# privacy-scaling-explorations/snark-verifier

Hardware: AMD Instinct MI355X
Metric: BN254 G1 MSM points/sec at 2^20 (higher is better)
Workload: dtype i32x9 (254-bit Montgomery Fq as 9 x 29-bit limbs on the integer VALU)

## Files before the change

snark-verifier_amd/csrc/ctx.hpp:

```cpp
#pragma once
#include <hip/hip_runtime.h>
#include <stddef.h>
#include <stdint.h>
#include <stdio.h>
#include "../../include/snarkv_amd.h"
#include "curve_consts.h"

#if defined(SNARKV_CURVE_PALLAS)
#define SNARKV_API(name) snarkv_pallas_##name
#else
#define SNARKV_API(name) snarkv_##name
#endif

namespace snarkv {

void set_last_error(const char* fmt, ...);

#define SNARKV_HIP(expr)                                                                   \
  do {                                                                                     \
    hipError_t _e = (expr);                                                                \
    if (_e != hipSuccess) {                                                                \
      ::snarkv::set_last_error("%s:%d: %s -> %s", __FILE__, __LINE__, #expr, hipGetErrorString(_e)); \
      return SNARKV_ERR_DEVICE;                                                            \
    }                                                                                      \
  } while (0)

#define SNARKV_TRY(expr)      \
  do {                        \
    int _rc = (expr);         \
    if (_rc < 0) return _rc;  \
  } while (0)

enum Slot {
  SLOT_IN_SCALARS = 0,
  SLOT_IN_POINTS,
  SLOT_IN_OFFSETS,
  SLOT_OUT,
  SLOT_POINTS_MONT,
  SLOT_COUNTS,
  SLOT_OFFSETS,
  SLOT_CURSOR,
  SLOT_BLOCKSUMS,
  SLOT_ENTRIES,
  SLOT_SEG_IDS,
  SLOT_SEG_PARTIALS,
  SLOT_BUCKETS,
  SLOT_CHUNK_PARTIALS,
  SLOT_WINDOW_SUMS,
  SLOT_TERM_PARTIALS,
  SLOT_FLAGS,
  SLOT_MISC,
  SLOT_SORT_TMP,
  SLOT_SHIFTED,
  SLOT_GLV,
  SLOT_BIG_LIST,
  SLOT_MISC2,
  SLOT_TERM_CHAIN,
  SLOT_TERM_MAGS,
  SLOT_SPLIT_PARTIALS,
  SLOT_IPA_XI,
  SLOT_IPA_H,
  SLOT_IPA_OUT,
  SLOT_MGPU_GRID,
  SLOT_MGPU_RECV,
  SLOT_COUNT
};

}

struct snarkv_ctx {
  int device;
  hipStream_t stream;
  bool own_stream;
  void* buf[snarkv::SLOT_COUNT];
  size_t cap[snarkv::SLOT_COUNT];
  void* hbuf[SNARKV_HOST_BUFFERS];
  size_t hbuf_cap[SNARKV_HOST_BUFFERS];
  uint32_t flags;
  bool mont;
  bool stage_timing;
  float stage_ms[SNARKV_PIP_STAGES];
  hipEvent_t ev[SNARKV_PIP_STAGES + 1];
  bool ev_ready;
  snarkv_ctx* sub[4];
  hipEvent_t sub_ev[5];
  bool sub_ready;
  hipEvent_t sorted_ev;
  bool sorted_ev_ready;
  int last_split_workers;
  bool throughput_mode;
  int throughput_peers;
  bool is_lane;
  snarkv_ctx* jobs[SNARKV_MANY_MAX_JOBS];
  int njobs;
  int last_many_jobs;
  size_t many_sig;
  hipStream_t copy_stream;
  bool copy_ready;
  hipEvent_t many_ev[2];
  hipEvent_t order_ev;
  bool order_ev_ready;
  hipStream_t hi_stream[2];
  bool hi_ready;
};

struct snarkv_dk {
  int device;
  void* d_prep;
// ... 66 lines not shown
```

snark-verifier_amd/csrc/msm_pippenger.hip:

```cpp
#include <stdlib.h>
#include <string.h>
#include <algorithm>
#include <mutex>
#include <atomic>
#include "ctx.hpp"
#include "g1_29.h"
#include "fr29.h"
#ifndef SNARKV_GLV
#define SNARKV_GLV 1
#endif
#if SNARKV_GLV
#include "glv.h"
#endif

namespace snarkv {

#ifndef SNARKV_KRUN
#define SNARKV_KRUN 64
#endif
#ifndef SNARKV_KCHUNK
#define SNARKV_KCHUNK 8
#endif
#ifndef SNARKV_TILE_THREADS
#define SNARKV_TILE_THREADS 256
#endif
#ifndef SNARKV_SCATTER_ATTR
#define SNARKV_SCATTER_ATTR __attribute__((amdgpu_waves_per_eu(5)))
#endif
#ifndef SNARKV_L2_THREADS
#define SNARKV_L2_THREADS 512
#endif
#ifndef SNARKV_LEVEL2_ATTR
#define SNARKV_LEVEL2_ATTR
#endif
#ifndef SNARKV_PREP_THREADS
#define SNARKV_PREP_THREADS SNARKV_TILE_THREADS
#endif
#ifndef SNARKV_XCD_TILES
#define SNARKV_XCD_TILES 1
#endif
#ifndef SNARKV_TILE_BASE
#define SNARKV_TILE_BASE 2048
#endif
#ifndef SNARKV_ACC_WAVES
#define SNARKV_ACC_WAVES 3
#endif
#ifndef SNARKV_BPRIO
#define SNARKV_BPRIO 3
#endif
#define SNARKV_RAISE_PRIO() __builtin_amdgcn_s_setprio(SNARKV_BPRIO)

constexpr int kHalves = SNARKV_GLV ? 2 : 1;
constexpr int kDigitWords = SNARKV_GLV ? 4 : 8;
constexpr int kDigitBits = 32 * kDigitWords;
constexpr int kRun = SNARKV_KRUN;
#ifndef SNARKV_KRUN_THROUGHPUT
#define SNARKV_KRUN_THROUGHPUT 96
#endif
constexpr int kRunThroughput = SNARKV_KRUN_THROUGHPUT;
constexpr int kChunk = SNARKV_KCHUNK;
constexpr uint32_t kSortCap = 7168;
constexpr uint32_t kSortTarget = 3072;
constexpr uint32_t kMaxKeys = 16384;
constexpr uint32_t kBigSpan = 24;
constexpr uint32_t kBigGrid = 8192;
constexpr uint32_t kMaxBig = 8192;
constexpr uint32_t kNoBucket = 0xFFFFFFFFu;

struct PipParams {
  uint32_t n;
  int c;
  int W;
  uint32_t B;
  uint32_t nb;
  int low_bits;
  uint32_t SB;
  uint32_t nkeys;
  uint32_t nblk;
  uint32_t tile;
  uint32_t mstride;
  uint32_t w0;
  uint32_t krun;
  uint32_t wper;
  uint32_t chunk_log2;
  uint32_t mont;
};

__device__ __forceinline__ uint32_t half_bits(const uint32_t (&k)[kDigitWords], int lo, int c) {
  if (lo >= kDigitBits) return 0;
  int word = lo >> 5, sh = lo & 31;
  uint32_t w0 = 0u, w1 = 0u;
#pragma unroll
  for (int i = 0; i < kDigitWords; ++i) {
    w0 = word == i ? k[i] : w0;
    if (i > 0) w1 = word == i - 1 ? k[i] : w1;
  }
  uint64_t v = ((uint64_t)w1 << 32) | w0;
  return (uint32_t)(v >> sh) & ((1u << c) - 1u);
}

template <class F>
__device__ __forceinline__ void for_each_digit(const uint32_t (&k)[kDigitWords], uint32_t sgn, const PipParams& p, F emit) {
  uint32_t carry = 0;
  for (int w = 0; w < p.W; ++w) {
    uint32_t raw = half_bits(k, w * p.c, p.c) + carry;
    uint32_t neg = raw > p.B ? 1u : 0u;
    uint32_t d = neg ? ((1u << p.c) - raw) : raw;
    carry = neg;
    if (d != 0) emit((uint32_t)w * p.SB + ((d - 1) >> p.low_bits), (uint32_t)w * p.B + d - 1, neg ^ sgn);
  }
}
template <class F>
__device__ __forceinline__ void digit_of_window(const uint32_t (&k)[kDigitWords], uint32_t sgn, const PipParams& p, int w,
                                                F emit) {
  uint32_t carry = 0;
  for (int j = w - 1; j >= 0; --j) {
    uint32_t b = half_bits(k, j * p.c, p.c);
    if (b != p.B) {
      carry = b > p.B ? 1u : 0u;
      break;
// ... 256 lines not shown
  SNARKV_RAISE_PRIO();
  extern __shared__ uint32_t lds[];
  const uint32_t nbins = 1u << p.low_bits;
  uint32_t* hist = lds;
  uint32_t* scan = lds + nbins;
  uint2* stage = reinterpret_cast<uint2*>(lds + nbins + SNARKV_L2_THREADS + (nbins & 1u));
  const uint32_t T = blockDim.x;
  uint32_t key = blockIdx.x;
  uint32_t begin = M[(size_t)key * p.mstride];
  uint32_t end = (key + 1 < p.nkeys) ? M[(size_t)(key + 1) * p.mstride] : misc[0];
  uint32_t cnt_items = end - begin;
  bool fast = cnt_items <= kSortCap;
  for (uint32_t k = threadIdx.x; k < nbins; k += T) hist[k] = 0;
  __syncthreads();
  const uint32_t low_mask = nbins - 1;
  constexpr int kPer = kSortCap / SNARKV_L2_THREADS;
  static_assert(kSortCap % SNARKV_L2_THREADS == 0, "kSortCap items spread evenly over the lanes");
  uint2 mine[kPer];
  if (fast) {
#pragma unroll
    for (int j = 0; j < kPer; ++j) {
      uint32_t e = threadIdx.x + j * T;
      if (e < cnt_items) {
        mine[j] = tmp[begin + e];
        atomicAdd(&hist[mine[j].x & low_mask], 1u);
      }
    }
  } else {
    for (uint32_t e = begin + threadIdx.x; e < end; e += T) atomicAdd(&hist[tmp[e].x & low_mask], 1u);
  }
  __syncthreads();
  uint32_t per = (nbins + T - 1) / T;
  uint32_t s0 = threadIdx.x * per;
  uint32_t sum = 0;
  for (uint32_t k = s0; k < s0 + per && k < nbins; ++k) sum += hist[k];
  scan[threadIdx.x] = sum;
  __syncthreads();
  for (uint32_t off = 1; off < T; off <<= 1) {
    uint32_t t = (threadIdx.x >= off) ? scan[threadIdx.x - off] : 0;
    __syncthreads();
    scan[threadIdx.x] += t;
    __syncthreads();
  }
  uint32_t run = scan[threadIdx.x] - sum;
  uint32_t w = key / p.SB, sb = key % p.SB;
  uint32_t bucket0 = w * p.B + (sb << p.low_bits);
  for (uint32_t k = s0; k < s0 + per && k < nbins; ++k) {
    uint32_t cnt = hist[k];
    counts[bucket0 + k] = cnt;
    offsets[bucket0 + k] = begin + run;
    hist[k] = run;
    run += cnt;
  }
  if (key == p.nkeys - 1 && threadIdx.x == 0) misc[4] = 0u;
  __syncthreads();
  if (fast) {
#pragma unroll
    for (int j = 0; j < kPer; ++j) {
      uint32_t e = threadIdx.x + j * T;
      if (e < cnt_items) stage[atomicAdd(&hist[mine[j].x & low_mask], 1u)] = mine[j];
    }
    __syncthreads();
    for (uint32_t e = threadIdx.x; e < cnt_items; e += T) entries[begin + e] = stage[e];
  } else {
    for (uint32_t e = begin + threadIdx.x; e < end; e += T) {
      uint2 it = tmp[e];
      entries[begin + atomicAdd(&hist[it.x & low_mask], 1u)] = it;
    }
  }
}

constexpr uint32_t kEntryIdx = 0x7FFFFFFFu;

__device__ __forceinline__ G1Affine29 entry_point(const G1Packed& k, uint32_t y) {
  G1Affine29 p = g1a29_unpack(k);
  if (y >> 31) p.y = fq29_neg(p.y);
  return p;
}

template <int RUN>
__global__ void __launch_bounds__(64, SNARKV_ACC_WAVES)
    k_accumulate(const uint2* __restrict__ entries, const uint32_t* __restrict__ total_ptr,
                 const G1Packed* __restrict__ pts, G1Xyzz29* __restrict__ buckets, uint32_t* __restrict__ seg_ids,
                 G1Xyzz29* __restrict__ seg_parts) {
  const uint32_t t = blockIdx.x * blockDim.x + threadIdx.x;
  const uint32_t stop = *total_ptr;
  const uint64_t begin64 = (uint64_t)t * RUN;
  if (begin64 >= stop) return;
  const uint32_t begin = (uint32_t)begin64;
  const uint32_t end = (stop - begin > (uint32_t)RUN) ? begin + RUN : stop;
  const size_t slot = t;
  uint32_t cur = entries[begin].x;
  bool first = true, fresh = true;
  G1Xyzz29 acc = xyzz29_identity();
  auto flush = [&]() {
    if (first) {
      seg_ids[2 * slot] = cur;
      seg_parts[2 * slot] = acc;
      first = false;
    } else {
      buckets[cur] = acc;
    }
  };
  auto step = [&](const uint2& ent, const G1Packed& pk) {
    if (ent.x != cur) {
      flush();
      cur = ent.x;
      fresh = true;
    }
    G1Affine29 p = entry_point(pk, ent.y);
    if (fresh) {
      acc.x = p.x;
      acc.y = p.y;
      acc.zz = fq29_one();
      acc.zzz = fq29_one();
      fresh = false;
    } else {
      xyzz29_madd_fast(acc, p);
    }
  };
  uint2 ent0 = entries[begin], ent1 = ent0;
  G1Packed p0 = pts[ent0.y & kEntryIdx], p1 = p0;
#pragma unroll 1
  for (uint32_t e = begin; e < end; e += 2) {
    if (e + 1 < end) {
      ent1 = entries[e + 1];
      p1 = pts[ent1.y & kEntryIdx];
    }
    step(ent0, p0);
    if (e + 1 < end) {
      if (e + 2 < end) {
        ent0 = entries[e + 2];
        p0 = pts[ent0.y & kEntryIdx];
      }
      step(ent1, p1);
    }
  }
  if (first) {
    seg_ids[2 * slot] = cur;
    seg_parts[2 * slot] = acc;
    seg_ids[2 * slot + 1] = kNoBucket;
  } else {
    seg_ids[2 * slot + 1] = cur;
    seg_parts[2 * slot + 1] = acc;
  }
}

__device__ __noinline__ void bucket_from_entries_careful(const uint2* __restrict__ entries, const G1Packed* __restrict__ pts,
                                                         uint32_t o, uint32_t cnt, uint32_t first, uint32_t stride,
                                                         bool sanitize, G1Xyzz29* out) {
  G1Xyzz29 acc = xyzz29_identity();
  for (uint32_t e = o + first; e < o + cnt; e += stride) {
    uint2 ent = entries[e];
    G1Affine29 p = entry_point(pts[ent.y & kEntryIdx], ent.y);
    xyzz29_madd_careful(acc, p);
  }
  *out = sanitize ? xyzz29_sanitize(acc) : acc;
}

__device__ __forceinline__ void run_span(const PipParams& p, uint32_t o, uint32_t cnt, size_t& s0, size_t& s1) {
  s0 = o / p.krun;
  s1 = (o + cnt - 1) / p.krun;
}

__global__ void __launch_bounds__(64)
    k_combine(const uint32_t* __restrict__ counts, const uint32_t* __restrict__ offsets, PipParams p,
              const uint2* __restrict__ entries, const G1Packed* __restrict__ pts,
              const uint32_t* __restrict__ seg_ids, const G1Xyzz29* __restrict__ seg_parts,
              G1Xyzz29* __restrict__ buckets, uint32_t* __restrict__ big_count, uint32_t* __restrict__ big_list) {
  SNARKV_RAISE_PRIO();
  uint32_t b = blockIdx.x * blockDim.x + threadIdx.x;
  if (b >= p.nb) return;
  uint32_t cnt = counts[b];
  if (cnt == 0) {
    buckets[b] = xyzz29_identity();
    return;
  }
  uint32_t o = offsets[b];
  size_t s0, s1;
  run_span(p, o, cnt, s0, s1);
  if (s1 - s0 >= kBigSpan) {
    uint32_t slot = atomicAdd(big_count, 1u);
    if (slot < kMaxBig) {
      big_list[slot] = b;
      return;
    }
  }
  G1Xyzz29 acc = xyzz29_identity();
  bool touched = false, bad = false;
  for (size_t s = s0; s <= s1; ++s) {
    for (int h = 0; h < 2; ++h) {
      if (seg_ids[2 * s + h] == b) {
        G1Xyzz29 part = seg_parts[2 * s + h];
        bad = bad || xyzz29_is_identity(part);
        xyzz29_add_skipid_fast(acc, part, bad);
        touched = true;
      }
    }
  }
  if (!touched) acc = buckets[b];
  bad = bad || xyzz29_is_degenerate(acc);
  if (bad) bucket_from_entries_careful(entries, pts, o, cnt, 0, 1, true, &buckets[b]);
  else if (touched) buckets[b] = acc;
}

__global__ void __launch_bounds__(256)
    k_combine_big(const uint32_t* __restrict__ counts, const uint32_t* __restrict__ offsets,
                  const uint2* __restrict__ entries, const G1Packed* __restrict__ pts,
                  const uint32_t* __restrict__ seg_ids, const G1Xyzz29* __restrict__ seg_parts,
                  G1Xyzz29* __restrict__ buckets, const uint32_t* __restrict__ big_count,
                  const uint32_t* __restrict__ big_list, PipParams p) {
  SNARKV_RAISE_PRIO();
  __shared__ G1Xyzz29 sh[256];
  __shared__ int any_bad;
  uint32_t nbig = *big_count < kMaxBig ? *big_count : kMaxBig;
  for (uint32_t bi = blockIdx.x; bi < nbig; bi += gridDim.x) {
    uint32_t b = big_list[bi];
    uint32_t o = offsets[b], cnt = counts[b];
    size_t s0, s1;
    run_span(p, o, cnt, s0, s1);
    if (threadIdx.x == 0) any_bad = 0;
    __syncthreads();
    G1Xyzz29 acc = xyzz29_identity();
    bool bad = false;
    for (size_t s = s0 + threadIdx.x; s <= s1; s += 256)
      for (int h = 0; h < 2; ++h)
        if (seg_ids[2 * s + h] == b) {
          G1Xyzz29 part = seg_parts[2 * s + h];
          bad = bad || xyzz29_is_degenerate(part);
          xyzz29_add_careful(acc, part);
        }
    if (bad) atomicOr(&any_bad, 1);
    __syncthreads();
    if (any_bad) bucket_from_entries_careful(entries, pts, o, cnt, threadIdx.x, 256, false, &sh[threadIdx.x]);
    else sh[threadIdx.x] = acc;
    __syncthreads();
    for (uint32_t st = 128; st >= 1; st >>= 1) {
      if (threadIdx.x < st) {
        G1Xyzz29 a = sh[threadIdx.x];
        xyzz29_add_careful(a, sh[threadIdx.x + st]);
        sh[threadIdx.x] = a;
      }
      __syncthreads();
    }
    if (threadIdx.x == 0) buckets[b] = xyzz29_sanitize(sh[0]);
    __syncthreads();
  }
}

__device__ __forceinline__ G1Xyzz29 xyzz29_sel(bool c, const G1Xyzz29& a, const G1Xyzz29& b) {
  G1Xyzz29 r;
#pragma unroll
  for (int i = 0; i < 9; ++i) {
    r.x.v[i] = c ? a.x.v[i] : b.x.v[i];
    r.y.v[i] = c ? a.y.v[i] : b.y.v[i];
    r.zz.v[i] = c ? a.zz.v[i] : b.zz.v[i];
    r.zzz.v[i] = c ? a.zzz.v[i] : b.zzz.v[i];
  }
  return r;
}

template <bool CAREFUL>
__device__ __forceinline__ bool chunk_sums(const G1Xyzz29* __restrict__ bw, uint32_t base, uint32_t top,
                                           G1Xyzz29& run, G1Xyzz29& acc) {
  run = xyzz29_identity();
  acc = xyzz29_identity();
  bool bad = false;
#pragma unroll 1
  for (uint32_t op = 0; op < 2 * (top - base); ++op) {
    bool second = op & 1u;
    G1Xyzz29 x = second ? acc : run;
    G1Xyzz29 y = second ? run : bw[top - 1 - (op >> 1)];
    if (CAREFUL) xyzz29_add_careful(x, y);
    else xyzz29_add_skipid_fast(x, y, bad);
    if (second) acc = x;
    else run = x;
  }
  if (CAREFUL) return false;
  return bad || (!xyzz29_is_identity(run) && xyzz29_is_degenerate(run)) ||
         (!xyzz29_is_identity(acc) && xyzz29_is_degenerate(acc));
}

__device__ __forceinline__ void wave_weighted_fold(G1Xyzz29* sh, const G1Xyzz29& run, const G1Xyzz29& acc,
                                                   const G1Xyzz29& extra, int log2_l, int log2_scale,
                                                   G1Xyzz29& out, G1Xyzz29* total_dst) {
  const uint32_t lane = threadIdx.x;
  G1Xyzz29 x = run;
#pragma unroll 1
  for (int step = 0; step < 14; ++step) {
    sh[lane] = x;
    __syncthreads();
    G1Xyzz29 y;
    int ndbl = 0;
    if (step == 6) {
      if (lane == 0 && total_dst) *total_dst = sh[0];
      x = xyzz29_sel(lane >= 1, x, xyzz29_identity());
      y = acc;
      ndbl = log2_l;
    } else if (step == 7) {
// ... 102 lines not shown
    }
    __syncthreads();
  }
  if (lane == 0) {
    if (partial_out) {
      *reinterpret_cast<G1Xyzz29*>(out) = sh[0];
    } else {
      G1Affine29 r = xyzz29_to_affine(sh[0]);
      uint32_t w[16];
      g1a29_to_words(r, w, mont != 0);
      for (int i = 0; i < 16; ++i) out[i] = w[i];
    }
  }
}

int launch_fold_partials_many(snarkv_ctx* ctx, const void* d_partials, size_t count, size_t jobs, void* d_out64s) {
  hipLaunchKernelGGL(k_final, dim3((uint32_t)jobs), dim3(64), 0, ctx->stream, (const G1Xyzz29*)d_partials, (uint32_t)count,
                     (uint32_t*)d_out64s, 0, ctx->mont ? 1u : 0u);
  SNARKV_HIP(hipGetLastError());
  return SNARKV_OK;
}

int launch_fold_partials(snarkv_ctx* ctx, const void* d_partials, size_t count, void* d_out64, bool partial_out) {
  hipLaunchKernelGGL(k_final, dim3(1), dim3(64), 0, ctx->stream, (const G1Xyzz29*)d_partials, (uint32_t)count,
                     (uint32_t*)d_out64, partial_out ? 1 : 0, ctx->mont ? 1u : 0u);
  SNARKV_HIP(hipGetLastError());
  return SNARKV_OK;
}

static int default_window_bits(size_t n) {
  int best = 2;
  double best_cost = 0;
  for (int c = 2; c <= 22; ++c) {
    const int W = (kDigitBits + c - 1) / c;
    const int top = kDigitBits - 1 - (W - 1) * c;
    double cost = (double)kHalves * (double)n * W * 10.0 + (double)W * (double)(1u << (c - 1)) * 30.0;
    if (top < c - 3) cost *= 1.6;
    if (c == 2 || cost < best_cost) best = c, best_cost = cost;
  }
  return best;
}

static int balance_window_bits(int c) {
  int W = (kDigitBits + c - 1) / c;
  return (kDigitBits + W - 1) / W;
}

static uint32_t latency_run_length(uint64_t entries) {
  auto waves = [&](uint64_t run) { return (entries + 64 * run - 1) / (64 * run); };
  if (waves(16) <= 4608) return waves(16) >= 2048 ? 16u : 32u;
  if (waves(32) <= 4608) return 32u;
  return (uint32_t)kRun;
}

int launch_msm_pippenger(snarkv_ctx* ctx, const void* d_scalars, const void* d_points, size_t n, int window_bits,
                         void* d_out, bool partial_out, void* d_buckets_out) {
  return launch_msm_pippenger_phases(ctx, ctx->stream, PIP_PHASE_ALL, d_scalars, d_points, n, window_bits, d_out,
                                     partial_out, d_buckets_out, nullptr);
}

int launch_msm_pippenger_phases(snarkv_ctx* ctx, hipStream_t st, int phases, const void* d_scalars, const void* d_points,
                                size_t n, int window_bits, void* d_out, bool partial_out, void* d_buckets_out,
                                void* d_grid) {
  PipParams p;
  p.w0 = 0;
  p.wper = 0;
  p.chunk_log2 = (uint32_t)kLog2Chunk;
  p.mont = ctx->mont ? 1u : 0u;
  p.n = (uint32_t)n;
  p.c = window_bits > 0 ? window_bits : balance_window_bits(default_window_bits(n));
  if (p.c < 2) p.c = 2;
  if (p.c > 22) p.c = 22;
  p.W = (kDigitBits + p.c - 1) / p.c;
  p.B = 1u << (p.c - 1);
  p.nb = (uint32_t)p.W * p.B;
  int high = p.c - 1 > 10 ? p.c - 1 - 10 : 0;
  while (high < p.c - 1 && ((kHalves * n) >> (high + 1)) >= kSortTarget && ((uint64_t)p.W << (high + 1)) <= kMaxKeys) ++high;
  p.low_bits = (p.c - 1) - high;
  p.SB = p.B >> p.low_bits;
  p.nkeys = (uint32_t)p.W * p.SB;
  p.tile = SNARKV_TILE_BASE;
  static_assert(kStageItems * kHalves <= 32, "a staged lane keeps one sign bit per entry in a 32-bit word");
  const size_t lds_staged = ((size_t)3 * p.SB + 16 + (p.SB & 1u)) * 4 + (size_t)kStageScalars * kHalves * 8;
  p.nblk = (uint32_t)((n + p.tile - 1) / p.tile);
  p.mstride = p.nblk | 1u;
  uint64_t max_entries = (uint64_t)kHalves * (uint64_t)n * (uint64_t)p.W;
  if (n == 0 || max_entries >= 0xFFFFFFFFull || n >= 0x40000000ull) {
    set_last_error("pippenger: n=%zu out of range", n);
    return SNARKV_ERR_LENGTH;
  }
  if ((size_t)p.nkeys * 4 > 65536 || lds_staged > 96 * 1024) {
    set_last_error("pippenger: key table too large (nkeys=%u)", p.nkeys);
    return SNARKV_ERR_LENGTH;
  }
  p.krun = ctx->throughput_mode ? (uint32_t)kRunThroughput : latency_run_length(max_entries);
  const uint32_t max_runs = (uint32_t)((max_entries + p.krun - 1) / p.krun) + 1;
  uint32_t mcount = p.nkeys * p.mstride;
  uint32_t scan_blocks = (mcount + 1023) / 1024;
  uint32_t chunks_per_window = (p.B + kChunk - 1) / kChunk;
  uint32_t blocks_per_window = (chunks_per_window + 63) / 64;

  void *d_pts, *d_glv, *d_counts, *d_offsets, *d_M, *d_blocksum, *d_entries, *d_tmp, *d_seg_ids, *d_seg_parts,
      *d_buckets, *d_wave, *d_shift, *d_misc, *d_big;
  SNARKV_TRY(ctx_reserve(ctx, SLOT_POINTS_MONT, kHalves * n * sizeof(G1Packed), &d_pts));
  SNARKV_TRY(ctx_reserve(ctx, SLOT_GLV, n * 32, &d_glv));
  SNARKV_TRY(ctx_reserve(ctx, SLOT_COUNTS, (size_t)p.nb * 4, &d_counts));
  SNARKV_TRY(ctx_reserve(ctx, SLOT_OFFSETS, (size_t)p.nb * 4, &d_offsets));
  SNARKV_TRY(ctx_reserve(ctx, SLOT_CURSOR, (size_t)mcount * 4, &d_M));
  SNARKV_TRY(ctx_reserve(ctx, SLOT_BLOCKSUMS, (size_t)scan_blocks * 4 + 64, &d_blocksum));
  SNARKV_TRY(ctx_reserve(ctx, SLOT_ENTRIES, max_entries * 8, &d_entries));
  SNARKV_TRY(ctx_reserve(ctx, SLOT_SORT_TMP, max_entries * 8, &d_tmp));
  SNARKV_TRY(ctx_reserve(ctx, SLOT_SEG_IDS, (size_t)max_runs * 8, &d_seg_ids));
  SNARKV_TRY(ctx_reserve(ctx, SLOT_SEG_PARTIALS, (size_t)max_runs * 2 * sizeof(G1Xyzz29), &d_seg_parts));
  if (d_grid) d_buckets = d_grid;
  else SNARKV_TRY(ctx_reserve(ctx, SLOT_BUCKETS, (size_t)p.nb * sizeof(G1Xyzz29), &d_buckets));
  SNARKV_TRY(ctx_reserve(ctx, SLOT_CHUNK_PARTIALS, 2 * (size_t)blocks_per_window * p.W * sizeof(G1Xyzz29), &d_wave));
  SNARKV_TRY(ctx_reserve(ctx, SLOT_SHIFTED, (size_t)p.W * sizeof(G1Xyzz29), &d_shift));
  SNARKV_TRY(ctx_reserve(ctx, SLOT_MISC, 64, &d_misc));
  SNARKV_TRY(ctx_reserve(ctx, SLOT_BIG_LIST, (size_t)kMaxBig * 4, &d_big));
  uint32_t* d_total = (uint32_t*)d_misc;
  uint32_t* d_big_count = d_total + 4;

  const bool tm = ctx->stage_timing && phases == PIP_PHASE_ALL;
  const bool tm_acc = ctx->stage_timing && phases == PIP_PHASE_ACC;
  int evi = 0;
#define STAGE_MARK()                                         \
  do {                                                       \
    if (tm) SNARKV_HIP(hipEventRecord(ctx->ev[evi++], st));  \
  } while (0)
  if ((tm || tm_acc) && !ctx->ev_ready) {
    for (int i = 0; i <= SNARKV_PIP_STAGES; ++i) SNARKV_HIP(hipEventCreate(&ctx->ev[i]));
    ctx->ev_ready = true;
  }
  STAGE_MARK();
  if (phases & PIP_PHASE_SORT) {
    hipLaunchKernelGGL(k_prepare, dim3(p.nblk), dim3(SNARKV_PREP_THREADS), (size_t)p.nkeys * 4, st, (const uint32_t*)d_scalars,
                       (const uint32_t*)d_points, (G1Packed*)d_pts, (uint4*)d_glv, p, (uint32_t*)d_M);
    STAGE_MARK();
    hipLaunchKernelGGL(k_scan_local, dim3(scan_blocks), dim3(256), 0, st, (uint32_t*)d_M, (uint32_t*)d_blocksum, mcount);
    hipLaunchKernelGGL(k_scan_blocksums, dim3(1), dim3(1024), 0, st, (uint32_t*)d_blocksum, scan_blocks, d_total);
    hipLaunchKernelGGL(k_scan_add, dim3(scan_blocks), dim3(256), 0, st, (uint32_t*)d_M, (const uint32_t*)d_blocksum,
                       mcount);
    STAGE_MARK();
    static std::atomic<uint64_t> attr_set{0};
    const uint64_t bit = 1ull << (ctx->device & 63);
    if (!(attr_set.load(std::memory_order_relaxed) & bit)) {
      SNARKV_HIP(hipFuncSetAttribute(reinterpret_cast<const void*>(k_sort_scatter_staged),
                                     hipFuncAttributeMaxDynamicSharedMemorySize, 96 * 1024));
      attr_set.fetch_or(bit, std::memory_order_relaxed);
    }
    hipLaunchKernelGGL(k_sort_scatter_staged, dim3(p.nblk), dim3(SNARKV_TILE_THREADS), lds_staged, st, (const uint4*)d_glv,
                       p, (const uint32_t*)d_M, (uint2*)d_tmp);
    const uint32_t nbins_l2 = 1u << p.low_bits;
    const size_t lds2 = ((size_t)nbins_l2 + SNARKV_L2_THREADS + 1) * 4 + (size_t)kSortCap * 8;
    hipLaunchKernelGGL(k_sort_level2, dim3(p.nkeys), dim3(SNARKV_L2_THREADS), lds2, st, (const uint2*)d_tmp, (const uint32_t*)d_M,
                       d_total, p, (uint2*)d_entries, (uint32_t*)d_counts, (uint32_t*)d_offsets);
  }
  STAGE_MARK();
  if (tm_acc) SNARKV_HIP(hipEventRecord(ctx->ev[3], st));
  if (phases & PIP_PHASE_ACC) {
    auto acc_kernel = p.krun == 16u ? k_accumulate<16> : p.krun == 32u ? k_accumulate<32>
                      : p.krun == (uint32_t)kRun ? k_accumulate<kRun> : k_accumulate<kRunThroughput>;
    hipLaunchKernelGGL(acc_kernel, dim3((max_runs + 63) / 64), dim3(64), 0, st, (const uint2*)d_entries,
                       (const uint32_t*)d_total, (const G1Packed*)d_pts, (G1Xyzz29*)d_buckets, (uint32_t*)d_seg_ids,
                       (G1Xyzz29*)d_seg_parts);
  }
  STAGE_MARK();
  if (tm_acc) SNARKV_HIP(hipEventRecord(ctx->ev[4], st));
  if (phases & PIP_PHASE_ACC) {
    hipLaunchKernelGGL(k_combine, dim3((p.nb + 63) / 64), dim3(64), 0, st, (const uint32_t*)d_counts,
                       (const uint32_t*)d_offsets, p, (const uint2*)d_entries, (const G1Packed*)d_pts,
                       (const uint32_t*)d_seg_ids, (const G1Xyzz29*)d_seg_parts, (G1Xyzz29*)d_buckets, d_big_count,
                       (uint32_t*)d_big);
    const uint32_t big_grid = std::min<uint32_t>(max_runs / kBigSpan + 1, kBigGrid);
    hipLaunchKernelGGL(k_combine_big, dim3(big_grid), dim3(256), 0, st, (const uint32_t*)d_counts,
                       (const uint32_t*)d_offsets, (const uint2*)d_entries, (const G1Packed*)d_pts,
                       (const uint32_t*)d_seg_ids, (const G1Xyzz29*)d_seg_parts, (G1Xyzz29*)d_buckets,
                       (const uint32_t*)d_big_count, (const uint32_t*)d_big, p);
    if (tm_acc) SNARKV_HIP(hipEventRecord(ctx->ev[5], st));
  }
  STAGE_MARK();
  if (d_buckets_out) {
    if (phases & PIP_PHASE_ACC)
      SNARKV_HIP(hipMemcpyAsync(d_buckets_out, d_buckets, (size_t)p.nb * sizeof(G1Xyzz29), hipMemcpyDeviceToDevice, st));
    SNARKV_HIP(hipGetLastError());
    return SNARKV_OK;
  }
  if (phases & PIP_PHASE_TAIL)
    hipLaunchKernelGGL(k_bucket_reduce, dim3(blocks_per_window * p.W), dim3(64), 0, st, (const G1Xyzz29*)d_buckets,
                       (G1Xyzz29*)d_wave, p, chunks_per_window, blocks_per_window);
  STAGE_MARK();
  if (phases & PIP_PHASE_TAIL)
    hipLaunchKernelGGL(k_shift_windows, dim3(p.W), dim3(64), 0, st, (const G1Xyzz29*)d_wave, (G1Xyzz29*)d_shift, p,
                       blocks_per_window);
  STAGE_MARK();
  if (phases & PIP_PHASE_TAIL)
    hipLaunchKernelGGL(k_final, dim3(1), dim3(64), 0, st, (const G1Xyzz29*)d_shift, (uint32_t)p.W, (uint32_t*)d_out,
                       partial_out ? 1 : 0, p.mont);
  STAGE_MARK();
#undef STAGE_MARK
  SNARKV_HIP(hipGetLastError());
  return SNARKV_OK;
}

int pip_geometry(size_t n_total, int window_bits, uint32_t* c, uint32_t* windows, uint32_t* buckets_per_window) {
  int cc = window_bits > 0 ? window_bits : balance_window_bits(default_window_bits(n_total));
  if (cc < 2) cc = 2;
  if (cc > 22) cc = 22;
  *c = (uint32_t)cc;
  *windows = (uint32_t)((kDigitBits + cc - 1) / cc);
  *buckets_per_window = 1u << (cc - 1);
  return SNARKV_OK;
}

__global__ void __launch_bounds__(256) k_buckets_add(G1Xyzz29* __restrict__ dst, const G1Xyzz29* __restrict__ src, uint32_t count) {
  SNARKV_RAISE_PRIO();
  uint32_t i = blockIdx.x * blockDim.x + threadIdx.x;
  if (i >= count) return;
  G1Xyzz29 a = dst[i];
  xyzz29_add_careful(a, src[i]);
  dst[i] = xyzz29_sanitize(a);
}

int launch_buckets_add(snarkv_ctx* ctx, void* d_dst, const void* d_src, size_t count) {
  hipLaunchKernelGGL(k_buckets_add, dim3((uint32_t)((count + 255) / 256)), dim3(256), 0, ctx->stream, (G1Xyzz29*)d_dst,
                     (const G1Xyzz29*)d_src, (uint32_t)count);
  SNARKV_HIP(hipGetLastError());
  return SNARKV_OK;
}

int launch_buckets_reduce(snarkv_ctx* ctx, const void* d_buckets, uint32_t c, uint32_t w0, uint32_t wcount,
// ... 80 lines not shown
```

Before: 762.9 million.

## Schedule bucket accumulation as length-sorted pieces instead of fixed entry runs

Replaces the fixed-length run accumulation (each thread handling RUN consecutive sorted entries that straddle buckets) with a piece schedule. Each bucket becomes whole or L-sized pieces, bucketed by length through a histogram plus scan, so the threads in a wave get similar trip counts and whole buckets write straight to the bucket array without the combine pass. A unified fixup kernel merges split buckets and recomputes degenerate ones. Run lengths are also raised to 128. The cost is extra histogram, scan and emit launches, plus more divergence-dependent padding within a wave.

```diff
diff --git a/snark-verifier_amd/csrc/ctx.hpp b/snark-verifier_amd/csrc/ctx.hpp
--- a/snark-verifier_amd/csrc/ctx.hpp
+++ b/snark-verifier_amd/csrc/ctx.hpp
@@ -42,8 +42,9 @@
   SLOT_CURSOR,
   SLOT_BLOCKSUMS,
   SLOT_ENTRIES,
-  SLOT_SEG_IDS,
-  SLOT_SEG_PARTIALS,
+  SLOT_PIECES,
+  SLOT_SPLIT_PARTS,
+  SLOT_PIECE_HIST,
   SLOT_BUCKETS,
   SLOT_CHUNK_PARTIALS,
   SLOT_WINDOW_SUMS,
@@ -53,7 +54,7 @@
   SLOT_SORT_TMP,
   SLOT_SHIFTED,
   SLOT_GLV,
-  SLOT_BIG_LIST,
+  SLOT_FIX_LISTS,
   SLOT_MISC2,
   SLOT_TERM_CHAIN,
   SLOT_TERM_MAGS,
diff --git a/snark-verifier_amd/csrc/msm_pippenger.hip b/snark-verifier_amd/csrc/msm_pippenger.hip
--- a/snark-verifier_amd/csrc/msm_pippenger.hip
+++ b/snark-verifier_amd/csrc/msm_pippenger.hip
@@ -16,7 +16,7 @@
 namespace snarkv {
 
 #ifndef SNARKV_KRUN
-#define SNARKV_KRUN 64
+#define SNARKV_KRUN 128
 #endif
 #ifndef SNARKV_KCHUNK
 #define SNARKV_KCHUNK 8
@@ -55,17 +55,13 @@
 constexpr int kDigitBits = 32 * kDigitWords;
 constexpr int kRun = SNARKV_KRUN;
 #ifndef SNARKV_KRUN_THROUGHPUT
-#define SNARKV_KRUN_THROUGHPUT 96
+#define SNARKV_KRUN_THROUGHPUT 128
 #endif
 constexpr int kRunThroughput = SNARKV_KRUN_THROUGHPUT;
 constexpr int kChunk = SNARKV_KCHUNK;
 constexpr uint32_t kSortCap = 7168;
 constexpr uint32_t kSortTarget = 3072;
 constexpr uint32_t kMaxKeys = 16384;
-constexpr uint32_t kBigSpan = 24;
-constexpr uint32_t kBigGrid = 8192;
-constexpr uint32_t kMaxBig = 8192;
-constexpr uint32_t kNoBucket = 0xFFFFFFFFu;
 
 struct PipParams {
   uint32_t n;
@@ -428,7 +424,6 @@
     hist[k] = run;
     run += cnt;
   }
-  if (key == p.nkeys - 1 && threadIdx.x == 0) misc[4] = 0u;
   __syncthreads();
   if (fast) {
 #pragma unroll
@@ -446,6 +441,64 @@
   }
 }
 
+constexpr uint32_t kSchedBuckets = 2048;
+constexpr uint32_t kMaxPiece = 256;
+constexpr uint32_t kBigPieces = 24;
+constexpr uint32_t kFixGrid = 1024;
+constexpr uint32_t kPieceWhole = 0x80000000u;
+__host__ __device__ constexpr uint32_t sched_rows(uint32_t L) { return L + 3; }
+
+__global__ void __launch_bounds__(256)
+    k_piece_hist(const uint32_t* __restrict__ counts, PipParams p, uint32_t nsb, uint32_t* __restrict__ H,
+                 uint32_t* __restrict__ misc) {
+  SNARKV_RAISE_PRIO();
+  __shared__ uint32_t hist[sched_rows(kMaxPiece)];
+  const uint32_t L = p.krun, rows = sched_rows(L);
+  for (uint32_t k = threadIdx.x; k < rows; k += blockDim.x) hist[k] = 0u;
+  if (blockIdx.x == 0 && threadIdx.x == 0) misc[4] = 0u;
+  __syncthreads();
+  const uint32_t lo = blockIdx.x * kSchedBuckets, hi = lo + kSchedBuckets < p.nb ? lo + kSchedBuckets : p.nb;
+  for (uint32_t b = lo + threadIdx.x; b < hi; b += blockDim.x) {
+    const uint32_t c = counts[b];
+    if (c <= L) {
+      atomicAdd(&hist[L - c], 1u);
+      continue;
+    }
+    const uint32_t nfull = c / L, r = c - nfull * L;
+    atomicAdd(&hist[0], nfull);
+    if (r) atomicAdd(&hist[L - r], 1u);
+    atomicAdd(&hist[nfull + (r ? 1u : 0u) > kBigPieces ? L + 2 : L + 1], 1u);
+  }
+  __syncthreads();
+  for (uint32_t k = threadIdx.x; k < rows; k += blockDim.x) H[(size_t)k * nsb + blockIdx.x] = hist[k];
+}
+
+__global__ void __launch_bounds__(256)
+    k_piece_emit(const uint32_t* __restrict__ counts, const uint32_t* __restrict__ offsets, PipParams p, uint32_t nsb,
+                 const uint32_t* __restrict__ H, uint32_t split_slots, uint4* __restrict__ pieces,
+                 uint32_t* __restrict__ small_list, uint32_t* __restrict__ big_list) {
+  SNARKV_RAISE_PRIO();
+  __shared__ uint32_t cur[sched_rows(kMaxPiece)];
+  const uint32_t L = p.krun, rows = sched_rows(L);
+  for (uint32_t k = threadIdx.x; k < rows; k += blockDim.x) cur[k] = H[(size_t)k * nsb + blockIdx.x];
+  const uint32_t small0 = H[(size_t)(L + 1) * nsb], big0 = H[(size_t)(L + 2) * nsb];
+  __syncthreads();
+  const uint32_t lo = blockIdx.x * kSchedBuckets, hi = lo + kSchedBuckets < p.nb ? lo + kSchedBuckets : p.nb;
+  for (uint32_t b = lo + threadIdx.x; b < hi; b += blockDim.x) {
+    const uint32_t c = counts[b], o = offsets[b];
+    if (c <= L) {
+      pieces[atomicAdd(&cur[L - c], 1u)] = make_uint4(o, c | kPieceWhole, b, 0u);
+      continue;
+    }
+    const uint32_t nfull = c / L, r = c - nfull * L, slot = o / L;
+    const uint32_t at = atomicAdd(&cur[0], nfull);
+    for (uint32_t j = 0; j < nfull; ++j) pieces[at + j] = make_uint4(o + j * L, L, b, slot + j);
+    if (r) pieces[atomicAdd(&cur[L - r], 1u)] = make_uint4(o + nfull * L, r, b, split_slots + slot);
+    if (nfull + (r ? 1u : 0u) > kBigPieces) big_list[atomicAdd(&cur[L + 2], 1u) - big0] = b;
+    else small_list[atomicAdd(&cur[L + 1], 1u) - small0] = b;
+  }
+}
+
 constexpr uint32_t kEntryIdx = 0x7FFFFFFFu;
 
 __device__ __forceinline__ G1Affine29 entry_point(const G1Packed& k, uint32_t y) {
@@ -454,71 +507,65 @@
   return p;
 }
 
-template <int RUN>
 __global__ void __launch_bounds__(64, SNARKV_ACC_WAVES)
-    k_accumulate(const uint2* __restrict__ entries, const uint32_t* __restrict__ total_ptr,
-                 const G1Packed* __restrict__ pts, G1Xyzz29* __restrict__ buckets, uint32_t* __restrict__ seg_ids,
-                 G1Xyzz29* __restrict__ seg_parts) {
-  const uint32_t t = blockIdx.x * blockDim.x + threadIdx.x;
+    k_accumulate(const uint4* __restrict__ pieces, const uint32_t* __restrict__ npieces_ptr,
+                 const uint32_t* __restrict__ total_ptr, const uint2* __restrict__ entries,
+                 const G1Packed* __restrict__ pts, G1Xyzz29* __restrict__ buckets, G1Xyzz29* __restrict__ parts,
+                 uint32_t part_slots, uint32_t* __restrict__ deg_count, uint32_t* __restrict__ deg_list, PipParams p) {
+  const uint32_t npieces = *npieces_ptr;
+  if (blockIdx.x * 64u >= npieces) return;
+  const uint32_t t = blockIdx.x * 64u + threadIdx.x;
   const uint32_t stop = *total_ptr;
-  const uint64_t begin64 = (uint64_t)t * RUN;
-  if (begin64 >= stop) return;
-  const uint32_t begin = (uint32_t)begin64;
-  const uint32_t end = (stop - begin > (uint32_t)RUN) ? begin + RUN : stop;
-  const size_t slot = t;
-  uint32_t cur = entries[begin].x;
-  bool first = true, fresh = true;
+  uint4 d = make_uint4(0u, 0u, 0u, 0u);
+  if (t < npieces) d = pieces[t];
+  const uint32_t first = d.x, b = d.z;
+  uint32_t len = d.y & ~kPieceWhole;
+  const bool whole = (d.y & kPieceWhole) != 0;
+  const bool valid = t < npieces && b < p.nb && len <= p.krun && first <= stop && len <= stop - first &&
+                     (whole || d.w < part_slots);
+  if (!valid) len = 0;
+  uint32_t trip = len;
+#pragma unroll
+  for (int off = 32; off >= 1; off >>= 1) trip = max(trip, (uint32_t)__shfl_xor((int)trip, off, 64));
+  trip = __builtin_amdgcn_readfirstlane(trip);
+  const uint32_t last = len ? first + len - 1 : 0u, nvirt = (uint32_t)kHalves * p.n;
+  uint2 ent0, ent1;
+  G1Packed p0, p1;
+  auto fetch = [&](uint32_t e, uint2& ent, G1Packed& pk) {
+    ent = entries[min(first + e, last)];
+    pk = pts[min(ent.y & kEntryIdx, nvirt - 1u)];
+  };
   G1Xyzz29 acc = xyzz29_identity();
-  auto flush = [&]() {
-    if (first) {
-      seg_ids[2 * slot] = cur;
-      seg_parts[2 * slot] = acc;
-      first = false;
-    } else {
-      buckets[cur] = acc;
-    }
-  };
-  auto step = [&](const uint2& ent, const G1Packed& pk) {
-    if (ent.x != cur) {
-      flush();
-      cur = ent.x;
-      fresh = true;
-    }
-    G1Affine29 p = entry_point(pk, ent.y);
-    if (fresh) {
-      acc.x = p.x;
-      acc.y = p.y;
+  fetch(0, ent0, p0);
+  if (trip) {
+    fetch(1, ent1, p1);
+    if (len) {
+      const G1Affine29 q = entry_point(p0, ent0.y);
+      acc.x = q.x;
+      acc.y = q.y;
       acc.zz = fq29_one();
       acc.zzz = fq29_one();
-      fresh = false;
-    } else {
-      xyzz29_madd_fast(acc, p);
-    }
-  };
-  uint2 ent0 = entries[begin], ent1 = ent0;
-  G1Packed p0 = pts[ent0.y & kEntryIdx], p1 = p0;
+    }
+  }
 #pragma unroll 1
-  for (uint32_t e = begin; e < end; e += 2) {
-    if (e + 1 < end) {
-      ent1 = entries[e + 1];
-      p1 = pts[ent1.y & kEntryIdx];
-    }
-    step(ent0, p0);
-    if (e + 1 < end) {
-      if (e + 2 < end) {
-        ent0 = entries[e + 2];
-        p0 = pts[ent0.y & kEntryIdx];
-      }
-      step(ent1, p1);
-    }
-  }
-  if (first) {
-    seg_ids[2 * slot] = cur;
-    seg_parts[2 * slot] = acc;
-    seg_ids[2 * slot + 1] = kNoBucket;
+  for (uint32_t e = 1; e < trip; e += 2) {
+    fetch(e + 1, ent0, p0);
+    if (e < len) xyzz29_madd_fast(acc, entry_point(p1, ent1.y));
+    if (e + 1 < trip) {
+      fetch(e + 2, ent1, p1);
+      if (e + 1 < len) xyzz29_madd_fast(acc, entry_point(p0, ent0.y));
+    }
+  }
+  if (!valid) return;
+  if (!whole) {
+    parts[d.w] = acc;
+  } else if (len == 0) {
+    buckets[b] = xyzz29_identity();
+  } else if (xyzz29_is_degenerate(acc)) {
+    const uint32_t i = atomicAdd(deg_count, 1u);
+    if (i < p.nb) deg_list[i] = b;
   } else {
-    seg_ids[2 * slot + 1] = cur;
-    seg_parts[2 * slot + 1] = acc;
+    buckets[b] = acc;
   }
 }
 
@@ -534,81 +581,38 @@
   *out = sanitize ? xyzz29_sanitize(acc) : acc;
 }
 
-__device__ __forceinline__ void run_span(const PipParams& p, uint32_t o, uint32_t cnt, size_t& s0, size_t& s1) {
-  s0 = o / p.krun;
-  s1 = (o + cnt - 1) / p.krun;
-}
-
-__global__ void __launch_bounds__(64)
-    k_combine(const uint32_t* __restrict__ counts, const uint32_t* __restrict__ offsets, PipParams p,
-              const uint2* __restrict__ entries, const G1Packed* __restrict__ pts,
-              const uint32_t* __restrict__ seg_ids, const G1Xyzz29* __restrict__ seg_parts,
-              G1Xyzz29* __restrict__ buckets, uint32_t* __restrict__ big_count, uint32_t* __restrict__ big_list) {
-  SNARKV_RAISE_PRIO();
-  uint32_t b = blockIdx.x * blockDim.x + threadIdx.x;
-  if (b >= p.nb) return;
-  uint32_t cnt = counts[b];
-  if (cnt == 0) {
-    buckets[b] = xyzz29_identity();
-    return;
-  }
-  uint32_t o = offsets[b];
-  size_t s0, s1;
-  run_span(p, o, cnt, s0, s1);
-  if (s1 - s0 >= kBigSpan) {
-    uint32_t slot = atomicAdd(big_count, 1u);
-    if (slot < kMaxBig) {
-      big_list[slot] = b;
-      return;
-    }
-  }
-  G1Xyzz29 acc = xyzz29_identity();
-  bool touched = false, bad = false;
-  for (size_t s = s0; s <= s1; ++s) {
-    for (int h = 0; h < 2; ++h) {
-      if (seg_ids[2 * s + h] == b) {
-        G1Xyzz29 part = seg_parts[2 * s + h];
-        bad = bad || xyzz29_is_identity(part);
-        xyzz29_add_skipid_fast(acc, part, bad);
-        touched = true;
-      }
-    }
-  }
-  if (!touched) acc = buckets[b];
-  bad = bad || xyzz29_is_degenerate(acc);
-  if (bad) bucket_from_entries_careful(entries, pts, o, cnt, 0, 1, true, &buckets[b]);
-  else if (touched) buckets[b] = acc;
+__device__ __forceinline__ uint32_t piece_slot(uint32_t o, uint32_t j, uint32_t nfull, uint32_t L, uint32_t split_slots) {
+  return j < nfull ? o / L + j : split_slots + o / L;
 }
 
 __global__ void __launch_bounds__(256)
-    k_combine_big(const uint32_t* __restrict__ counts, const uint32_t* __restrict__ offsets,
-                  const uint2* __restrict__ entries, const G1Packed* __restrict__ pts,
-                  const uint32_t* __restrict__ seg_ids, const G1Xyzz29* __restrict__ seg_parts,
-                  G1Xyzz29* __restrict__ buckets, const uint32_t* __restrict__ big_count,
-                  const uint32_t* __restrict__ big_list, PipParams p) {
+    k_fixup(const uint32_t* __restrict__ counts, const uint32_t* __restrict__ offsets, const uint2* __restrict__ entries,
+            const G1Packed* __restrict__ pts, const G1Xyzz29* __restrict__ parts, uint32_t split_slots,
+            G1Xyzz29* __restrict__ buckets, const uint32_t* __restrict__ H, uint32_t nsb, const uint32_t* __restrict__ misc,
+            const uint32_t* __restrict__ small_list, const uint32_t* __restrict__ big_list,
+            const uint32_t* __restrict__ deg_list, PipParams p) {
   SNARKV_RAISE_PRIO();
   __shared__ G1Xyzz29 sh[256];
   __shared__ int any_bad;
-  uint32_t nbig = *big_count < kMaxBig ? *big_count : kMaxBig;
+  const uint32_t L = p.krun;
+  const uint32_t small0 = H[(size_t)(L + 1) * nsb], big0 = H[(size_t)(L + 2) * nsb];
+  const uint32_t nsmall = big0 - small0, nbig = misc[6] - big0;
+  const uint32_t ndeg = misc[4] < p.nb ? misc[4] : p.nb;
   for (uint32_t bi = blockIdx.x; bi < nbig; bi += gridDim.x) {
-    uint32_t b = big_list[bi];
-    uint32_t o = offsets[b], cnt = counts[b];
-    size_t s0, s1;
-    run_span(p, o, cnt, s0, s1);
+    const uint32_t b = big_list[bi];
+    const uint32_t o = offsets[b], cnt = counts[b], nfull = cnt / L, np = nfull + (cnt % L ? 1u : 0u);
     if (threadIdx.x == 0) any_bad = 0;
     __syncthreads();
     G1Xyzz29 acc = xyzz29_identity();
     bool bad = false;
-    for (size_t s = s0 + threadIdx.x; s <= s1; s += 256)
-      for (int h = 0; h < 2; ++h)
-        if (seg_ids[2 * s + h] == b) {
-          G1Xyzz29 part = seg_parts[2 * s + h];
-          bad = bad || xyzz29_is_degenerate(part);
-          xyzz29_add_careful(acc, part);
-        }
+    for (uint32_t j = threadIdx.x; j < np; j += blockDim.x) {
+      const G1Xyzz29 part = parts[piece_slot(o, j, nfull, L, split_slots)];
+      bad = bad || xyzz29_is_degenerate(part);
+      xyzz29_add_careful(acc, part);
+    }
     if (bad) atomicOr(&any_bad, 1);
     __syncthreads();
-    if (any_bad) bucket_from_entries_careful(entries, pts, o, cnt, threadIdx.x, 256, false, &sh[threadIdx.x]);
+    if (any_bad) bucket_from_entries_careful(entries, pts, o, cnt, threadIdx.x, blockDim.x, false, &sh[threadIdx.x]);
     else sh[threadIdx.x] = acc;
     __syncthreads();
     for (uint32_t st = 128; st >= 1; st >>= 1) {
@@ -621,6 +625,24 @@
     }
     if (threadIdx.x == 0) buckets[b] = xyzz29_sanitize(sh[0]);
     __syncthreads();
+  }
+  for (uint32_t i = blockIdx.x * blockDim.x + threadIdx.x; i < nsmall + ndeg; i += gridDim.x * blockDim.x) {
+    const bool split = i < nsmall;
+    const uint32_t b = split ? small_list[i] : deg_list[i - nsmall];
+    const uint32_t o = offsets[b], cnt = counts[b];
+    bool bad = !split;
+    G1Xyzz29 acc = xyzz29_identity();
+    if (split) {
+      const uint32_t nfull = cnt / L, np = nfull + (cnt % L ? 1u : 0u);
+      for (uint32_t j = 0; j < np; ++j) {
+        const G1Xyzz29 part = parts[piece_slot(o, j, nfull, L, split_slots)];
+        bad = bad || xyzz29_is_identity(part);
+        xyzz29_add_skipid_fast(acc, part, bad);
+      }
+      bad = bad || xyzz29_is_degenerate(acc);
+    }
+    if (bad) bucket_from_entries_careful(entries, pts, o, cnt, 0, 1, true, &buckets[b]);
+    else buckets[b] = acc;
   }
 }
 
@@ -829,6 +851,8 @@
   if (waves(32) <= 4608) return 32u;
   return (uint32_t)kRun;
 }
+static_assert(kRun >= 32 && kRun <= (int)kMaxPiece && kRunThroughput >= 16 && kRunThroughput <= (int)kMaxPiece,
+              "piece caps fit the schedule's LDS rows");
 
 int launch_msm_pippenger(snarkv_ctx* ctx, const void* d_scalars, const void* d_points, size_t n, int window_bits,
                          void* d_out, bool partial_out, void* d_buckets_out) {
@@ -871,32 +895,38 @@
     return SNARKV_ERR_LENGTH;
   }
   p.krun = ctx->throughput_mode ? (uint32_t)kRunThroughput : latency_run_length(max_entries);
-  const uint32_t max_runs = (uint32_t)((max_entries + p.krun - 1) / p.krun) + 1;
+  const uint32_t max_pieces = (uint32_t)std::min<uint64_t>((uint64_t)p.nb + max_entries / p.krun, 0xFFFFFFFFull - 63);
+  const uint32_t split_slots = (uint32_t)(max_entries / p.krun) + 1;
+  const uint32_t nsb = (p.nb + kSchedBuckets - 1) / kSchedBuckets;
+  const uint32_t hcount = sched_rows(p.krun) * nsb;
+  const uint32_t hscan_blocks = (hcount + 1023) / 1024;
   uint32_t mcount = p.nkeys * p.mstride;
   uint32_t scan_blocks = (mcount + 1023) / 1024;
   uint32_t chunks_per_window = (p.B + kChunk - 1) / kChunk;
   uint32_t blocks_per_window = (chunks_per_window + 63) / 64;
 
-  void *d_pts, *d_glv, *d_counts, *d_offsets, *d_M, *d_blocksum, *d_entries, *d_tmp, *d_seg_ids, *d_seg_parts,
-      *d_buckets, *d_wave, *d_shift, *d_misc, *d_big;
+  void *d_pts, *d_glv, *d_counts, *d_offsets, *d_M, *d_blocksum, *d_entries, *d_tmp, *d_pieces, *d_hist, *d_parts,
+      *d_buckets, *d_wave, *d_shift, *d_misc, *d_lists;
   SNARKV_TRY(ctx_reserve(ctx, SLOT_POINTS_MONT, kHalves * n * sizeof(G1Packed), &d_pts));
   SNARKV_TRY(ctx_reserve(ctx, SLOT_GLV, n * 32, &d_glv));
   SNARKV_TRY(ctx_reserve(ctx, SLOT_COUNTS, (size_t)p.nb * 4, &d_counts));
   SNARKV_TRY(ctx_reserve(ctx, SLOT_OFFSETS, (size_t)p.nb * 4, &d_offsets));
   SNARKV_TRY(ctx_reserve(ctx, SLOT_CURSOR, (size_t)mcount * 4, &d_M));
-  SNARKV_TRY(ctx_reserve(ctx, SLOT_BLOCKSUMS, (size_t)scan_blocks * 4 + 64, &d_blocksum));
+  SNARKV_TRY(ctx_reserve(ctx, SLOT_BLOCKSUMS, (size_t)std::max(scan_blocks, hscan_blocks) * 4 + 64, &d_blocksum));
   SNARKV_TRY(ctx_reserve(ctx, SLOT_ENTRIES, max_entries * 8, &d_entries));
   SNARKV_TRY(ctx_reserve(ctx, SLOT_SORT_TMP, max_entries * 8, &d_tmp));
-  SNARKV_TRY(ctx_reserve(ctx, SLOT_SEG_IDS, (size_t)max_runs * 8, &d_seg_ids));
-  SNARKV_TRY(ctx_reserve(ctx, SLOT_SEG_PARTIALS, (size_t)max_runs * 2 * sizeof(G1Xyzz29), &d_seg_parts));
+  SNARKV_TRY(ctx_reserve(ctx, SLOT_PIECES, (size_t)max_pieces * sizeof(uint4), &d_pieces));
+  SNARKV_TRY(ctx_reserve(ctx, SLOT_PIECE_HIST, (size_t)hcount * 4, &d_hist));
+  SNARKV_TRY(ctx_reserve(ctx, SLOT_SPLIT_PARTS, (size_t)split_slots * 2 * sizeof(G1Xyzz29), &d_parts));
   if (d_grid) d_buckets = d_grid;
   else SNARKV_TRY(ctx_reserve(ctx, SLOT_BUCKETS, (size_t)p.nb * sizeof(G1Xyzz29), &d_buckets));
   SNARKV_TRY(ctx_reserve(ctx, SLOT_CHUNK_PARTIALS, 2 * (size_t)blocks_per_window * p.W * sizeof(G1Xyzz29), &d_wave));
   SNARKV_TRY(ctx_reserve(ctx, SLOT_SHIFTED, (size_t)p.W * sizeof(G1Xyzz29), &d_shift));
   SNARKV_TRY(ctx_reserve(ctx, SLOT_MISC, 64, &d_misc));
-  SNARKV_TRY(ctx_reserve(ctx, SLOT_BIG_LIST, (size_t)kMaxBig * 4, &d_big));
+  SNARKV_TRY(ctx_reserve(ctx, SLOT_FIX_LISTS, (size_t)p.nb * 3 * 4, &d_lists));
   uint32_t* d_total = (uint32_t*)d_misc;
-  uint32_t* d_big_count = d_total + 4;
+  uint32_t* d_small = (uint32_t*)d_lists, *d_bigl = d_small + p.nb, *d_deg = d_bigl + p.nb;
+  const uint32_t* d_npieces = (const uint32_t*)d_hist + (size_t)(p.krun + 1) * nsb;
 
   const bool tm = ctx->stage_timing && phases == PIP_PHASE_ALL;
   const bool tm_acc = ctx->stage_timing && phases == PIP_PHASE_ACC;
@@ -932,28 +962,30 @@
     const size_t lds2 = ((size_t)nbins_l2 + SNARKV_L2_THREADS + 1) * 4 + (size_t)kSortCap * 8;
     hipLaunchKernelGGL(k_sort_level2, dim3(p.nkeys), dim3(SNARKV_L2_THREADS), lds2, st, (const uint2*)d_tmp, (const uint32_t*)d_M,
                        d_total, p, (uint2*)d_entries, (uint32_t*)d_counts, (uint32_t*)d_offsets);
+    hipLaunchKernelGGL(k_piece_hist, dim3(nsb), dim3(256), 0, st, (const uint32_t*)d_counts, p, nsb, (uint32_t*)d_hist,
+                       d_total);
+    hipLaunchKernelGGL(k_scan_local, dim3(hscan_blocks), dim3(256), 0, st, (uint32_t*)d_hist, (uint32_t*)d_blocksum, hcount);
+    hipLaunchKernelGGL(k_scan_blocksums, dim3(1), dim3(1024), 0, st, (uint32_t*)d_blocksum, hscan_blocks, d_total + 6);
+    hipLaunchKernelGGL(k_scan_add, dim3(hscan_blocks), dim3(256), 0, st, (uint32_t*)d_hist, (const uint32_t*)d_blocksum,
+                       hcount);
+    hipLaunchKernelGGL(k_piece_emit, dim3(nsb), dim3(256), 0, st, (const uint32_t*)d_counts, (const uint32_t*)d_offsets, p,
+                       nsb, (const uint32_t*)d_hist, split_slots, (uint4*)d_pieces, d_small, d_bigl);
   }
   STAGE_MARK();
   if (tm_acc) SNARKV_HIP(hipEventRecord(ctx->ev[3], st));
-  if (phases & PIP_PHASE_ACC) {
-    auto acc_kernel = p.krun == 16u ? k_accumulate<16> : p.krun == 32u ? k_accumulate<32>
-                      : p.krun == (uint32_t)kRun ? k_accumulate<kRun> : k_accumulate<kRunThroughput>;
-    hipLaunchKernelGGL(acc_kernel, dim3((max_runs + 63) / 64), dim3(64), 0, st, (const uint2*)d_entries,
-                       (const uint32_t*)d_total, (const G1Packed*)d_pts, (G1Xyzz29*)d_buckets, (uint32_t*)d_seg_ids,
-                       (G1Xyzz29*)d_seg_parts);
-  }
+  if (phases & PIP_PHASE_ACC)
+    hipLaunchKernelGGL(k_accumulate, dim3((max_pieces + 63) / 64), dim3(64), 0, st, (const uint4*)d_pieces, d_npieces,
+                       (const uint32_t*)d_total, (const uint2*)d_entries, (const G1Packed*)d_pts, (G1Xyzz29*)d_buckets,
+                       (G1Xyzz29*)d_parts, 2 * split_slots, d_total + 4, d_deg, p);
   STAGE_MARK();
   if (tm_acc) SNARKV_HIP(hipEventRecord(ctx->ev[4], st));
   if (phases & PIP_PHASE_ACC) {
-    hipLaunchKernelGGL(k_combine, dim3((p.nb + 63) / 64), dim3(64), 0, st, (const uint32_t*)d_counts,
-                       (const uint32_t*)d_offsets, p, (const uint2*)d_entries, (const G1Packed*)d_pts,
-                       (const uint32_t*)d_seg_ids, (const G1Xyzz29*)d_seg_parts, (G1Xyzz29*)d_buckets, d_big_count,
-                       (uint32_t*)d_big);
-    const uint32_t big_grid = std::min<uint32_t>(max_runs / kBigSpan + 1, kBigGrid);
-    hipLaunchKernelGGL(k_combine_big, dim3(big_grid), dim3(256), 0, st, (const uint32_t*)d_counts,
-                       (const uint32_t*)d_offsets, (const uint2*)d_entries, (const G1Packed*)d_pts,
-                       (const uint32_t*)d_seg_ids, (const G1Xyzz29*)d_seg_parts, (G1Xyzz29*)d_buckets,
-                       (const uint32_t*)d_big_count, (const uint32_t*)d_big, p);
+    const uint64_t split_bound = std::min<uint64_t>(p.nb, max_entries / (p.krun + 1) + 1);
+    const uint32_t fix_grid = (uint32_t)std::min<uint64_t>((split_bound + 255) / 256, kFixGrid);
+    hipLaunchKernelGGL(k_fixup, dim3(fix_grid), dim3(256), 0, st, (const uint32_t*)d_counts, (const uint32_t*)d_offsets,
+                       (const uint2*)d_entries, (const G1Packed*)d_pts, (const G1Xyzz29*)d_parts, split_slots,
+                       (G1Xyzz29*)d_buckets, (const uint32_t*)d_hist, nsb, (const uint32_t*)d_total,
+                       (const uint32_t*)d_small, (const uint32_t*)d_bigl, (const uint32_t*)d_deg, p);
     if (tm_acc) SNARKV_HIP(hipEventRecord(ctx->ev[5], st));
   }
   STAGE_MARK();
```

Result: faster. 815.6 million (median of 6 runs) (+6.9%).
